# EternityJune25/ComoRAG

Measured on NVIDIA H100. Metric: queries/sec, higher is better.
Workload: dtype bf16

## Files before the change

### comorag_b200/csrc/gemm.cu

```cuda
#include <cstdlib>

#include "common.cuh"
#include "gemm.cuh"
#include "ptx.cuh"

namespace crag {

constexpr int kGemmBM = 128;
constexpr int kGemmBN = 128;
constexpr int kGemmBK = 64;
constexpr int kGemmConsumerWarps = 8;
constexpr int kGemmThreads = 32 * kGemmConsumerWarps + 32;
constexpr int kGemmStages = 3;

struct GemmLayout {
  static constexpr int kABytes = kGemmBM * kGemmBK * 2;
  static constexpr int kBBytes = kGemmBN * kGemmBK * 2;
  static constexpr int kStageBytes = kABytes + kBBytes;
  static constexpr size_t smem_bytes() { return 1024 + size_t(kGemmStages) * kStageBytes + 2 * kGemmStages * 8; }
};

__device__ __forceinline__ float gelu_erf(float x) {
  const float z = x * 0.70710678118654752f;
  const float az = fabsf(z);
  float t;
  asm("rcp.approx.ftz.f32 %0, %1;" : "=f"(t) : "f"(fmaf(0.3275911f, az, 1.0f)));
  float p = fmaf(1.061405429f, t, -1.453152027f);
  p = fmaf(p, t, 1.421413741f);
  p = fmaf(p, t, -0.284496736f);
  p = fmaf(p, t, 0.254829592f);
  p *= t;
  float e;
  asm("ex2.approx.ftz.f32 %0, %1;" : "=f"(e) : "f"(az * az * -1.4426950408889634f));
  const float erf_abs = fmaf(-p, e, 1.0f);
  const float half_x = 0.5f * x;
  return fmaf(half_x, copysignf(erf_abs, z), half_x);
}

__device__ __forceinline__ uint32_t pack_bf16x2(float a, float b) {
  __nv_bfloat162 v = __floats2bfloat162_rn(a, b);
  return *reinterpret_cast<uint32_t*>(&v);
}

template <int EPI>
__global__ void __launch_bounds__(kGemmThreads, 2)
gemm_bf16_kernel(const __grid_constant__ CUtensorMap tm_a, const __grid_constant__ CUtensorMap tm_b, int M, int N,
                 int K, const float* __restrict__ bias, const __nv_bfloat16* __restrict__ residual, int64_t ldr,
                 __nv_bfloat16* __restrict__ out, int64_t ldo) {
  using L = GemmLayout;
  constexpr int STAGES = kGemmStages;
  extern __shared__ uint8_t smem_raw[];
  uint8_t* smem = reinterpret_cast<uint8_t*>((reinterpret_cast<uintptr_t>(smem_raw) + 1023) & ~uintptr_t(1023));
  uint64_t* bar_full = reinterpret_cast<uint64_t*>(smem + STAGES * L::kStageBytes);
  uint64_t* bar_empty = bar_full + STAGES;

  const int warp = threadIdx.x >> 5;
  const int lane = threadIdx.x & 31;
  const int n_blk = blockIdx.x, m_blk = blockIdx.y;
  const int num_kb = (K + kGemmBK - 1) / kGemmBK;

  if (threadIdx.x == 0) {
    for (int s = 0; s < STAGES; ++s) {
      mbar_init(&bar_full[s], 1);
      mbar_init(&bar_empty[s], kGemmConsumerWarps);
    }
    fence_mbar_init();
  }
  __syncthreads();

  if (warp == kGemmConsumerWarps) {
    if (lane == 0) {
      tma_prefetch_desc(&tm_a);
      tma_prefetch_desc(&tm_b);
      const uint64_t pol_w = policy_evict_last();
      int stage = 0;
      uint32_t phase = 0;
      for (int kb = 0; kb < num_kb; ++kb) {
        mbar_wait(&bar_empty[stage], phase ^ 1);
        uint8_t* sa = smem + stage * L::kStageBytes;
        mbar_arrive_expect_tx(&bar_full[stage], L::kStageBytes);
        tma_load_2d(&tm_a, &bar_full[stage], sa, kb * kGemmBK, m_blk * kGemmBM);
        tma_load_2d_hint(&tm_b, &bar_full[stage], sa + L::kABytes, kb * kGemmBK, n_blk * kGemmBN, pol_w);
        if (++stage == STAGES) { stage = 0; phase ^= 1; }
      }
    }
    return;
  }

  const int wg = warp >> 2;
  float acc[kGemmBN / 2];
#pragma unroll
  for (int i = 0; i < kGemmBN / 2; ++i) acc[i] = 0.f;
  int stage = 0, prev = 0;
  uint32_t phase = 0;
  for (int kb = 0; kb < num_kb; ++kb) {
    mbar_wait(&bar_full[stage], phase);
    const uint32_t a_addr = smem_u32(smem + stage * L::kStageBytes) + wg * 64 * 128;
    const uint32_t b_addr = smem_u32(smem + stage * L::kStageBytes + L::kABytes);
    wgmma_fence();
#pragma unroll
    for (int ks = 0; ks < kGemmBK / 16; ++ks)
      wgmma_m64n128k16_ss(acc, wgmma_desc_sw128(a_addr + ks * 32), wgmma_desc_sw128(b_addr + ks * 32), 1u);
    wgmma_commit();
    wgmma_wait<1>();
    if (kb > 0 && lane == 0) mbar_arrive(&bar_empty[prev]);
    prev = stage;
    if (++stage == STAGES) { stage = 0; phase ^= 1; }
  }
  wgmma_wait<0>();
  wgmma_fence_regs(acc);

  const int row0 = m_blk * kGemmBM + wg * 64 + (warp & 3) * 16 + (lane >> 2);
  const int col0 = n_blk * kGemmBN + 2 * (lane & 3);
#pragma unroll
  for (int j = 0; j < kGemmBN / 8; ++j) {
    const int col = col0 + 8 * j;
    if (col >= N) continue;
    const float2 b = __ldg(reinterpret_cast<const float2*>(bias + col));
#pragma unroll
    for (int h = 0; h < 2; ++h) {
      const int row = row0 + 8 * h;
      if (row >= M) continue;
      float x0 = acc[4 * j + 2 * h] + b.x, x1 = acc[4 * j + 2 * h + 1] + b.y;
      if (EPI == GEMM_EPI_BIAS_GELU) {
        x0 = gelu_erf(x0);
        x1 = gelu_erf(x1);
      }
      if (EPI == GEMM_EPI_BIAS_RESIDUAL) {
        const __nv_bfloat162 r = *reinterpret_cast<const __nv_bfloat162*>(residual + int64_t(row) * ldr + col);
        x0 += __bfloat162float(r.x);
        x1 += __bfloat162float(r.y);
      }
      *reinterpret_cast<uint32_t*>(out + int64_t(row) * ldo + col) = pack_bf16x2(x0, x1);
    }
  }
}

template <int EPI>
static int launch_gemm_t(const CUtensorMap& tm_a, const CUtensorMap& tm_b, int M, int N, int K, const float* bias,
                         const __nv_bfloat16* residual, int64_t ldr, __nv_bfloat16* out, int64_t ldo,
                         cudaStream_t stream) {
  auto kern = gemm_bf16_kernel<EPI>;
  {
    static bool done[64] = {false};
    int dev = 0;
    CRAG_CUDA_OK(cudaGetDevice(&dev));
    if (dev < 0 || dev >= 64 || !done[dev]) {
      CRAG_CUDA_OK(cudaFuncSetAttribute(kern, cudaFuncAttributeMaxDynamicSharedMemorySize, int(GemmLayout::smem_bytes())));
      if (dev >= 0 && dev < 64) done[dev] = true;
    }
  }
  const dim3 grid((N + kGemmBN - 1) / kGemmBN, (M + kGemmBM - 1) / kGemmBM);
  kern<<<grid, kGemmThreads, GemmLayout::smem_bytes(), stream>>>(tm_a, tm_b, M, N, K, bias, residual, ldr, out, ldo);
  CRAG_CUDA_OK(cudaGetLastError());
  return CRAG_OK;
}

int gemm_bf16(const void* a, int64_t lda, const void* w, int64_t ldw, const float* bias, const void* residual,
              int64_t ldr, void* out, int64_t ldo, int M, int N, int K, int epi, cudaStream_t stream) {
  if (M <= 0) return CRAG_OK;
  if (N < 8 || K < 8 || N % 8 != 0 || K % 8 != 0) return fail(CRAG_ERR_INVALID, "gemm: N and K must be positive multiples of 8 (N=%d K=%d)", N, K);
  if (lda % 8 || ldw % 8 || ldo % 8 || (epi == GEMM_EPI_BIAS_RESIDUAL && ldr % 8)) return fail(CRAG_ERR_INVALID, "gemm: leading dimensions must be multiples of 8 elements");
  if (!a || !w || !bias || !out || (epi == GEMM_EPI_BIAS_RESIDUAL && !residual)) return fail(CRAG_ERR_INVALID, "gemm: null pointer");
  if ((uintptr_t(a) | uintptr_t(w) | uintptr_t(out) | uintptr_t(bias) | uintptr_t(residual)) & 15) return fail(CRAG_ERR_INVALID, "gemm: pointers must be 16-byte aligned");
  if ((M + kGemmBM - 1) / kGemmBM > 65535) return fail(CRAG_ERR_INVALID, "gemm: M too large (%d)", M);
  const __nv_bfloat16* res = static_cast<const __nv_bfloat16*>(residual);
  __nv_bfloat16* o = static_cast<__nv_bfloat16*>(out);
  CUtensorMap tm_a, tm_b;
  int rc = make_tmap_bf16_2d(&tm_a, a, uint64_t(M), uint64_t(K), uint64_t(lda) * 2, kGemmBM);
  if (rc != CRAG_OK) return rc;
  rc = make_tmap_bf16_2d(&tm_b, w, uint64_t(N), uint64_t(K), uint64_t(ldw) * 2, kGemmBN);
  if (rc != CRAG_OK) return rc;
  switch (epi) {
    case GEMM_EPI_BIAS: return launch_gemm_t<GEMM_EPI_BIAS>(tm_a, tm_b, M, N, K, bias, res, ldr, o, ldo, stream);
    case GEMM_EPI_BIAS_GELU: return launch_gemm_t<GEMM_EPI_BIAS_GELU>(tm_a, tm_b, M, N, K, bias, res, ldr, o, ldo, stream);
    case GEMM_EPI_BIAS_RESIDUAL: return launch_gemm_t<GEMM_EPI_BIAS_RESIDUAL>(tm_a, tm_b, M, N, K, bias, res, ldr, o, ldo, stream);
  }
  return fail(CRAG_ERR_INVALID, "gemm: unknown epilogue %d", epi);
}

}

extern "C" int crag_gemm_bf16(const void* a, int64_t lda, const void* w, int64_t ldw, const float* bias,
                              const void* residual, int64_t ldr, void* out, int64_t ldo, int m, int n, int k,
                              int epilogue, crag_stream_t stream) {
  return crag::gemm_bf16(a, lda, w, ldw, bias, residual, ldr, out, ldo, m, n, k, epilogue,
                         static_cast<cudaStream_t>(stream));
}
```

### comorag_b200/csrc/ptx.cuh

```cuda
#pragma once
#include <cuda.h>
#include <cuda_runtime.h>
#include <cuda_bf16.h>
#include <stdint.h>

namespace crag {

__device__ __forceinline__ uint32_t smem_u32(const void* p) {
  return static_cast<uint32_t>(__cvta_generic_to_shared(p));
}

__device__ __forceinline__ bool elect_one() {
  uint32_t pred = 0;
  asm volatile(
      "{\n\t.reg .pred p;\n\t"
      "elect.sync _|p, 0xffffffff;\n\t"
      "selp.u32 %0, 1, 0, p;\n\t}"
      : "=r"(pred));
  return pred != 0;
}

__device__ __forceinline__ void mbar_init(uint64_t* bar, uint32_t count) {
  asm volatile("mbarrier.init.shared::cta.b64 [%0], %1;" ::"r"(smem_u32(bar)), "r"(count));
}
__device__ __forceinline__ void fence_mbar_init() {
  asm volatile("fence.mbarrier_init.release.cluster;" ::: "memory");
}
__device__ __forceinline__ void fence_proxy_async() {
  asm volatile("fence.proxy.async.shared::cta;" ::: "memory");
}
__device__ __forceinline__ void mbar_arrive_expect_tx(uint64_t* bar, uint32_t bytes) {
  asm volatile("mbarrier.arrive.expect_tx.shared::cta.b64 _, [%0], %1;" ::"r"(smem_u32(bar)), "r"(bytes)
               : "memory");
}
__device__ __forceinline__ void mbar_arrive(uint64_t* bar) {
  asm volatile("mbarrier.arrive.shared::cta.b64 _, [%0];" ::"r"(smem_u32(bar)) : "memory");
}
__device__ __forceinline__ bool mbar_try_wait(uint64_t* bar, uint32_t parity) {
  uint32_t ok;
  asm volatile(
      "{\n\t.reg .pred p;\n\t"
      "mbarrier.try_wait.parity.shared::cta.b64 p, [%1], %2;\n\t"
      "selp.u32 %0, 1, 0, p;\n\t}"
      : "=r"(ok)
      : "r"(smem_u32(bar)), "r"(parity)
      : "memory");
  return ok != 0;
}
#ifndef CRAG_MBAR_SPIN_LIMIT
#define CRAG_MBAR_SPIN_LIMIT (1ll << 33)
#endif
__device__ __forceinline__ void mbar_wait(uint64_t* bar, uint32_t parity) {
  if (mbar_try_wait(bar, parity)) return;
  const long long t0 = clock64();
  uint32_t spins = 0;
  while (!mbar_try_wait(bar, parity)) {
    if ((++spins & 0x3FF) == 0 && clock64() - t0 > CRAG_MBAR_SPIN_LIMIT) __trap();
  }
}

__device__ __forceinline__ void tma_prefetch_desc(const CUtensorMap* m) {
  asm volatile("prefetch.tensormap [%0];" ::"l"(reinterpret_cast<uint64_t>(m)) : "memory");
}
__device__ __forceinline__ void tma_load_2d(const CUtensorMap* m, uint64_t* bar, void* dst, int32_t c0,
                                            int32_t c1) {
  asm volatile(
      "cp.async.bulk.tensor.2d.shared::cluster.global.mbarrier::complete_tx::bytes"
      " [%0], [%1, {%3, %4}], [%2];" ::"r"(smem_u32(dst)),
      "l"(reinterpret_cast<uint64_t>(m)), "r"(smem_u32(bar)), "r"(c0), "r"(c1)
      : "memory");
}
__device__ __forceinline__ void tma_load_2d_hint(const CUtensorMap* m, uint64_t* bar, void* dst, int32_t c0,
                                                 int32_t c1, uint64_t policy) {
  asm volatile(
      "cp.async.bulk.tensor.2d.shared::cluster.global.mbarrier::complete_tx::bytes.L2::cache_hint"
      " [%0], [%1, {%3, %4}], [%2], %5;" ::"r"(smem_u32(dst)),
      "l"(reinterpret_cast<uint64_t>(m)), "r"(smem_u32(bar)), "r"(c0), "r"(c1), "l"(policy)
      : "memory");
}
__device__ __forceinline__ uint64_t policy_evict_first() {
  uint64_t p;
  asm volatile("createpolicy.fractional.L2::evict_first.b64 %0, 1.0;" : "=l"(p));
  return p;
}
__device__ __forceinline__ uint64_t policy_evict_normal() {
  uint64_t p;
  asm volatile("createpolicy.fractional.L2::evict_normal.b64 %0, 1.0;" : "=l"(p));
  return p;
}
__device__ __forceinline__ uint64_t policy_evict_last() {
  uint64_t p;
  asm volatile("createpolicy.fractional.L2::evict_last.b64 %0, 1.0;" : "=l"(p));
  return p;
}

__device__ __forceinline__ void wgmma_fence() { asm volatile("wgmma.fence.sync.aligned;" ::: "memory"); }
__device__ __forceinline__ void wgmma_commit() { asm volatile("wgmma.commit_group.sync.aligned;" ::: "memory"); }
template <int N>
__device__ __forceinline__ void wgmma_wait() { asm volatile("wgmma.wait_group.sync.aligned %0;" ::"n"(N) : "memory"); }
template <int R>
__device__ __forceinline__ void wgmma_fence_regs(float (&d)[R]) {
#pragma unroll
  for (int i = 0; i < R; ++i) asm volatile("" : "+f"(d[i])::"memory");
}

__device__ __forceinline__ uint64_t wgmma_desc_sw128(uint32_t smem_addr) {
  uint64_t d = 0;
  d |= static_cast<uint64_t>((smem_addr & 0x3FFFF) >> 4);
  d |= static_cast<uint64_t>(1) << 16;
  d |= static_cast<uint64_t>(1024 >> 4) << 32;
  d |= static_cast<uint64_t>(1) << 62;
  return d;
}

__device__ __forceinline__ void wgmma_m64n32k16_ss(float (&d)[16], uint64_t desc_a, uint64_t desc_b, uint32_t accumulate) {
  asm volatile(
      "{\n\t.reg .pred p;\n\t"
      "setp.ne.b32 p, %18, 0;\n\t"
      "wgmma.mma_async.sync.aligned.m64n32k16.f32.bf16.bf16 "
      "{%0, %1, %2, %3, %4, %5, %6, %7, %8, %9, %10, %11, %12, %13, %14, %15}, %16, %17, p, 1, 1, 0, 0;\n\t}"
      : "+f"(d[0]), "+f"(d[1]), "+f"(d[2]), "+f"(d[3]), "+f"(d[4]), "+f"(d[5]), "+f"(d[6]), "+f"(d[7]), "+f"(d[8]), "+f"(d[9]), "+f"(d[10]), "+f"(d[11]), "+f"(d[12]), "+f"(d[13]), "+f"(d[14]), "+f"(d[15])
      : "l"(desc_a), "l"(desc_b), "r"(accumulate));
}
__device__ __forceinline__ void wgmma_m64n64k16_ss(float (&d)[32], uint64_t desc_a, uint64_t desc_b, uint32_t accumulate) {
  asm volatile(
      "{\n\t.reg .pred p;\n\t"
      "setp.ne.b32 p, %34, 0;\n\t"
      "wgmma.mma_async.sync.aligned.m64n64k16.f32.bf16.bf16 "
      "{%0, %1, %2, %3, %4, %5, %6, %7, %8, %9, %10, %11, %12, %13, %14, %15, %16, %17, %18, %19, %20, %21, %22, %23, %24, %25, %26, %27, %28, %29, %30, %31}, %32, %33, p, 1, 1, 0, 0;\n\t}"
      : "+f"(d[0]), "+f"(d[1]), "+f"(d[2]), "+f"(d[3]), "+f"(d[4]), "+f"(d[5]), "+f"(d[6]), "+f"(d[7]), "+f"(d[8]), "+f"(d[9]), "+f"(d[10]), "+f"(d[11]), "+f"(d[12]), "+f"(d[13]), "+f"(d[14]), "+f"(d[15]), "+f"(d[16]), "+f"(d[17]), "+f"(d[18]), "+f"(d[19]), "+f"(d[20]), "+f"(d[21]), "+f"(d[22]), "+f"(d[23]), "+f"(d[24]), "+f"(d[25]), "+f"(d[26]), "+f"(d[27]), "+f"(d[28]), "+f"(d[29]), "+f"(d[30]), "+f"(d[31])
      : "l"(desc_a), "l"(desc_b), "r"(accumulate));
}
__device__ __forceinline__ void wgmma_m64n128k16_ss(float (&d)[64], uint64_t desc_a, uint64_t desc_b, uint32_t accumulate) {
  asm volatile(
      "{\n\t.reg .pred p;\n\t"
      "setp.ne.b32 p, %66, 0;\n\t"
      "wgmma.mma_async.sync.aligned.m64n128k16.f32.bf16.bf16 "
      "{%0, %1, %2, %3, %4, %5, %6, %7, %8, %9, %10, %11, %12, %13, %14, %15, %16, %17, %18, %19, %20, %21, %22, %23, %24, %25, %26, %27, %28, %29, %30, %31, %32, %33, %34, %35, %36, %37, %38, %39, %40, %41, %42, %43, %44, %45, %46, %47, %48, %49, %50, %51, %52, %53, %54, %55, %56, %57, %58, %59, %60, %61, %62, %63}, %64, %65, p, 1, 1, 0, 0;\n\t}"
      : "+f"(d[0]), "+f"(d[1]), "+f"(d[2]), "+f"(d[3]), "+f"(d[4]), "+f"(d[5]), "+f"(d[6]), "+f"(d[7]), "+f"(d[8]), "+f"(d[9]), "+f"(d[10]), "+f"(d[11]), "+f"(d[12]), "+f"(d[13]), "+f"(d[14]), "+f"(d[15]), "+f"(d[16]), "+f"(d[17]), "+f"(d[18]), "+f"(d[19]), "+f"(d[20]), "+f"(d[21]), "+f"(d[22]), "+f"(d[23]), "+f"(d[24]), "+f"(d[25]), "+f"(d[26]), "+f"(d[27]), "+f"(d[28]), "+f"(d[29]), "+f"(d[30]), "+f"(d[31]), "+f"(d[32]), "+f"(d[33]), "+f"(d[34]), "+f"(d[35]), "+f"(d[36]), "+f"(d[37]), "+f"(d[38]), "+f"(d[39]), "+f"(d[40]), "+f"(d[41]), "+f"(d[42]), "+f"(d[43]), "+f"(d[44]), "+f"(d[45]), "+f"(d[46]), "+f"(d[47]), "+f"(d[48]), "+f"(d[49]), "+f"(d[50]), "+f"(d[51]), "+f"(d[52]), "+f"(d[53]), "+f"(d[54]), "+f"(d[55]), "+f"(d[56]), "+f"(d[57]), "+f"(d[58]), "+f"(d[59]), "+f"(d[60]), "+f"(d[61]), "+f"(d[62]), "+f"(d[63])
      : "l"(desc_a), "l"(desc_b), "r"(accumulate));
}
__device__ __forceinline__ void wgmma_m64n64k16_rs_bmn(float (&d)[32], const uint32_t (&a)[4], uint64_t desc_b,
                                                      uint32_t accumulate) {
  asm volatile(
      "{\n\t.reg .pred p;\n\t"
      "setp.ne.b32 p, %37, 0;\n\t"
      "wgmma.mma_async.sync.aligned.m64n64k16.f32.bf16.bf16 "
      "{%0, %1, %2, %3, %4, %5, %6, %7, %8, %9, %10, %11, %12, %13, %14, %15, %16, %17, %18, %19, %20, %21, %22, %23, %24, %25, %26, %27, %28, %29, %30, %31}, {%32, %33, %34, %35}, %36, p, 1, 1, 1;\n\t}"
      : "+f"(d[0]), "+f"(d[1]), "+f"(d[2]), "+f"(d[3]), "+f"(d[4]), "+f"(d[5]), "+f"(d[6]), "+f"(d[7]), "+f"(d[8]), "+f"(d[9]), "+f"(d[10]), "+f"(d[11]), "+f"(d[12]), "+f"(d[13]), "+f"(d[14]), "+f"(d[15]), "+f"(d[16]), "+f"(d[17]), "+f"(d[18]), "+f"(d[19]), "+f"(d[20]), "+f"(d[21]), "+f"(d[22]), "+f"(d[23]), "+f"(d[24]), "+f"(d[25]), "+f"(d[26]), "+f"(d[27]), "+f"(d[28]), "+f"(d[29]), "+f"(d[30]), "+f"(d[31])
      : "r"(a[0]), "r"(a[1]), "r"(a[2]), "r"(a[3]), "l"(desc_b), "r"(accumulate));
}

__device__ __forceinline__ void named_bar_sync(uint32_t id, uint32_t nthreads) {
  asm volatile("barrier.cta.sync %0, %1;" ::"r"(id), "r"(nthreads) : "memory");
}
__device__ __forceinline__ bool named_bar_or(uint32_t id, uint32_t nthreads, bool pred) {
  uint32_t out;
  asm volatile(
      "{\n\t.reg .pred p, q;\n\t"
      "setp.ne.b32 p, %1, 0;\n\t"
      "barrier.cta.red.or.pred q, %2, %3, p;\n\t"
      "selp.u32 %0, 1, 0, q;\n\t}"
      : "=r"(out)
      : "r"(static_cast<uint32_t>(pred)), "r"(id), "r"(nthreads)
      : "memory");
  return out != 0;
}

}
```

Baseline: 4611.

## Add persistent warp-specialized 128x256 GEMM with TMA-store epilogue for large problems

Adds a persistent GEMM kernel with 128x256 tiles, used when the wide tile count is at least the SM count. It uses a grouped-M tile order for L2 reuse, register reallocation between the producer and the two consumer warpgroups, and an epilogue that stages output in swizzled shared memory, writes it with TMA stores, and TMA-loads the residual. The aim is better wgmma efficiency and operand reuse, lower launch and tail overhead, and less uncoalesced epilogue traffic. It costs one CTA per SM, heavy register pressure from 128 accumulators, and no overlap between the epilogue and the next tile's MMA within a warpgroup.

Result: no change. 4606 (median of 6 runs) (-0.1%).

```diff
diff --git a/comorag_b200/csrc/gemm.cu b/comorag_b200/csrc/gemm.cu
--- a/comorag_b200/csrc/gemm.cu
+++ b/comorag_b200/csrc/gemm.cu
@@ -136,6 +136,192 @@
   }
 }
 
+constexpr int kWideBN = 256;
+constexpr int kWideStages = 3;
+constexpr int kWideThreads = 384;
+constexpr int kGemmGroupM = 16;
+
+struct WideLayout {
+  static constexpr int kABytes = kGemmBM * kGemmBK * 2;
+  static constexpr int kBBytes = kWideBN * kGemmBK * 2;
+  static constexpr int kStageBytes = kABytes + kBBytes;
+  static constexpr int kOutBoxBytes = 64 * 64 * 2;
+  static constexpr int kOutBytes = 4 * kOutBoxBytes;
+  static constexpr int kOutOffset = kWideStages * kStageBytes;
+  static constexpr int kBarOffset = kOutOffset + 2 * kOutBytes;
+  static constexpr size_t smem_bytes() { return 1024 + size_t(kBarOffset) + (2 * kWideStages + 2) * 8; }
+};
+
+template <int EPI>
+__global__ void __launch_bounds__(kWideThreads, 1)
+gemm_bf16_persistent_kernel(const __grid_constant__ CUtensorMap tm_a, const __grid_constant__ CUtensorMap tm_b,
+                            const __grid_constant__ CUtensorMap tm_out, const __grid_constant__ CUtensorMap tm_res,
+                            int M, int N, int K, const float* __restrict__ bias) {
+  using L = WideLayout;
+  constexpr int STAGES = kWideStages;
+  extern __shared__ uint8_t smem_raw[];
+  uint8_t* smem = reinterpret_cast<uint8_t*>((reinterpret_cast<uintptr_t>(smem_raw) + 1023) & ~uintptr_t(1023));
+  uint64_t* bar_full = reinterpret_cast<uint64_t*>(smem + L::kBarOffset);
+  uint64_t* bar_empty = bar_full + STAGES;
+  uint64_t* bar_res = bar_empty + STAGES;
+
+  const int warp = threadIdx.x >> 5;
+  const int lane = threadIdx.x & 31;
+  const int num_kb = (K + kGemmBK - 1) / kGemmBK;
+  const int tiles_m = (M + kGemmBM - 1) / kGemmBM;
+  const int tiles_n = (N + kWideBN - 1) / kWideBN;
+  const int num_tiles = tiles_m * tiles_n;
+  auto tile_coords = [&](int tile, int& m_blk, int& n_blk) {
+    const int group = tile / (kGemmGroupM * tiles_n);
+    const int first_m = group * kGemmGroupM;
+    const int group_m = min(kGemmGroupM, tiles_m - first_m);
+    const int in_group = tile - group * kGemmGroupM * tiles_n;
+    m_blk = first_m + in_group % group_m;
+    n_blk = in_group / group_m;
+  };
+
+  if (threadIdx.x == 0) {
+    for (int s = 0; s < STAGES; ++s) {
+      mbar_init(&bar_full[s], 1);
+      mbar_init(&bar_empty[s], kGemmConsumerWarps);
+    }
+    mbar_init(&bar_res[0], 1);
+    mbar_init(&bar_res[1], 1);
+    fence_mbar_init();
+  }
+  __syncthreads();
+
+  if (warp < 4) {
+    setmaxnreg_dec<40>();
+    if (warp == 0 && lane == 0) {
+      tma_prefetch_desc(&tm_a);
+      tma_prefetch_desc(&tm_b);
+      const uint64_t pol_w = policy_evict_last();
+      int stage = 0;
+      uint32_t phase = 0;
+      for (int tile = blockIdx.x; tile < num_tiles; tile += gridDim.x) {
+        int m_blk, n_blk;
+        tile_coords(tile, m_blk, n_blk);
+        for (int kb = 0; kb < num_kb; ++kb) {
+          mbar_wait(&bar_empty[stage], phase ^ 1);
+          uint8_t* sa = smem + stage * L::kStageBytes;
+          mbar_arrive_expect_tx(&bar_full[stage], L::kStageBytes);
+          tma_load_2d(&tm_a, &bar_full[stage], sa, kb * kGemmBK, m_blk * kGemmBM);
+          tma_load_2d_hint(&tm_b, &bar_full[stage], sa + L::kABytes, kb * kGemmBK, n_blk * kWideBN, pol_w);
+          if (++stage == STAGES) { stage = 0; phase ^= 1; }
+        }
+      }
+    }
+    return;
+  }
+
+  setmaxnreg_inc<232>();
+  const int wg = (warp >> 2) - 1;
+  const bool leader = (threadIdx.x & 127) == 0;
+  uint8_t* out_tile = smem + L::kOutOffset + wg * L::kOutBytes;
+  const int frag_row = (warp & 3) * 16 + (lane >> 2);
+  const uint32_t frag_off = frag_row * 128 + 4 * (lane & 3);
+  const uint32_t swz = lane >> 2;
+  if (leader) {
+    tma_prefetch_desc(&tm_out);
+    if (EPI == GEMM_EPI_BIAS_RESIDUAL) tma_prefetch_desc(&tm_res);
+  }
+  int stage = 0;
+  uint32_t phase = 0, res_phase = 0;
+  float acc[kWideBN / 2];
+  for (int tile = blockIdx.x; tile < num_tiles; tile += gridDim.x) {
+    int m_blk, n_blk;
+    tile_coords(tile, m_blk, n_blk);
+    const int row0 = m_blk * kGemmBM + wg * 64, col0 = n_blk * kWideBN;
+    if (leader) {
+      bulk_wait_group_read<0>();
+      if (EPI == GEMM_EPI_BIAS_RESIDUAL) {
+        mbar_arrive_expect_tx(&bar_res[wg], L::kOutBytes);
+#pragma unroll
+        for (int b = 0; b < 4; ++b) tma_load_2d(&tm_res, &bar_res[wg], out_tile + b * L::kOutBoxBytes, col0 + 64 * b, row0);
+      }
+    }
+#pragma unroll
+    for (int i = 0; i < kWideBN / 2; ++i) acc[i] = 0.f;
+    int prev = 0;
+    for (int kb = 0; kb < num_kb; ++kb) {
+      mbar_wait(&bar_full[stage], phase);
+      const uint32_t a_addr = smem_u32(smem + stage * L::kStageBytes) + wg * 64 * 128;
+      const uint32_t b_addr = smem_u32(smem + stage * L::kStageBytes + L::kABytes);
+      wgmma_fence();
+#pragma unroll
+      for (int ks = 0; ks < kGemmBK / 16; ++ks)
+        wgmma_m64n256k16_ss(acc, wgmma_desc_sw128(a_addr + ks * 32), wgmma_desc_sw128(b_addr + ks * 32), 1u);
+      wgmma_commit();
+      wgmma_wait<1>();
+      if (kb > 0 && lane == 0) mbar_arrive(&bar_empty[prev]);
+      prev = stage;
+      if (++stage == STAGES) { stage = 0; phase ^= 1; }
+    }
+    wgmma_wait<0>();
+    wgmma_fence_regs(acc);
+    if (lane == 0) mbar_arrive(&bar_empty[prev]);
+
+    if (EPI == GEMM_EPI_BIAS_RESIDUAL) {
+      mbar_wait(&bar_res[wg], res_phase);
+      res_phase ^= 1;
+    } else {
+      named_bar_sync(1 + wg, 128);
+    }
+    const uint32_t out_base = smem_u32(out_tile) + frag_off;
+#pragma unroll
+    for (int j = 0; j < kWideBN / 8; ++j) {
+      const int col = col0 + 8 * j + 2 * (lane & 3);
+      const float2 b = col < N ? __ldg(reinterpret_cast<const float2*>(bias + col)) : make_float2(0.f, 0.f);
+      const uint32_t addr = out_base + (j >> 3) * L::kOutBoxBytes + (((j & 7) ^ swz) << 4);
+#pragma unroll
+      for (int h = 0; h < 2; ++h) {
+        float x0 = acc[4 * j + 2 * h] + b.x, x1 = acc[4 * j + 2 * h + 1] + b.y;
+        if (EPI == GEMM_EPI_BIAS_GELU) {
+          x0 = gelu_erf(x0);
+          x1 = gelu_erf(x1);
+        }
+        if (EPI == GEMM_EPI_BIAS_RESIDUAL) {
+          uint32_t rv;
+          asm volatile("ld.shared.b32 %0, [%1];" : "=r"(rv) : "r"(addr + h * 8 * 128));
+          const __nv_bfloat162 r = *reinterpret_cast<const __nv_bfloat162*>(&rv);
+          x0 += __bfloat162float(r.x);
+          x1 += __bfloat162float(r.y);
+        }
+        asm volatile("st.shared.b32 [%0], %1;" ::"r"(addr + h * 8 * 128), "r"(pack_bf16x2(x0, x1)) : "memory");
+      }
+    }
+    fence_proxy_async();
+    named_bar_sync(1 + wg, 128);
+    if (leader) {
+#pragma unroll
+      for (int b = 0; b < 4; ++b) tma_store_2d(&tm_out, out_tile + b * L::kOutBoxBytes, col0 + 64 * b, row0);
+      bulk_commit_group();
+    }
+  }
+  if (leader) bulk_wait_group_read<0>();
+}
+
+template <int EPI>
+static int launch_gemm_wide_t(const CUtensorMap& tm_a, const CUtensorMap& tm_b, const CUtensorMap& tm_out,
+                              const CUtensorMap& tm_res, int M, int N, int K, const float* bias, int num_tiles,
+                              int sms, cudaStream_t stream) {
+  auto kern = gemm_bf16_persistent_kernel<EPI>;
+  {
+    static bool done[64] = {false};
+    int dev = 0;
+    CRAG_CUDA_OK(cudaGetDevice(&dev));
+    if (dev < 0 || dev >= 64 || !done[dev]) {
+      CRAG_CUDA_OK(cudaFuncSetAttribute(kern, cudaFuncAttributeMaxDynamicSharedMemorySize, int(WideLayout::smem_bytes())));
+      if (dev >= 0 && dev < 64) done[dev] = true;
+    }
+  }
+  kern<<<min(num_tiles, sms), kWideThreads, WideLayout::smem_bytes(), stream>>>(tm_a, tm_b, tm_out, tm_res, M, N, K,
+                                                                               bias);
+  CRAG_CUDA_OK(cudaGetLastError());
+  return CRAG_OK;
+}
+
 template <int EPI>
 static int launch_gemm_t(const CUtensorMap& tm_a, const CUtensorMap& tm_b, int M, int N, int K, const float* bias,
                          const __nv_bfloat16* residual, int64_t ldr, __nv_bfloat16* out, int64_t ldo,
@@ -169,6 +355,27 @@
   CUtensorMap tm_a, tm_b;
   int rc = make_tmap_bf16_2d(&tm_a, a, uint64_t(M), uint64_t(K), uint64_t(lda) * 2, kGemmBM);
   if (rc != CRAG_OK) return rc;
+  const int sms = sm_count();
+  if (sms <= 0) return CRAG_ERR_CUDA;
+  const int wide_tiles = ((M + kGemmBM - 1) / kGemmBM) * ((N + kWideBN - 1) / kWideBN);
+  if (wide_tiles >= sms) {
+    CUtensorMap tm_out, tm_res;
+    rc = make_tmap_bf16_2d(&tm_b, w, uint64_t(N), uint64_t(K), uint64_t(ldw) * 2, kWideBN);
+    if (rc != CRAG_OK) return rc;
+    rc = make_tmap_bf16_2d(&tm_out, out, uint64_t(M), uint64_t(N), uint64_t(ldo) * 2, 64);
+    if (rc != CRAG_OK) return rc;
+    tm_res = tm_out;
+    if (epi == GEMM_EPI_BIAS_RESIDUAL) {
+      rc = make_tmap_bf16_2d(&tm_res, residual, uint64_t(M), uint64_t(N), uint64_t(ldr) * 2, 64);
+      if (rc != CRAG_OK) return rc;
+    }
+    switch (epi) {
+      case GEMM_EPI_BIAS: return launch_gemm_wide_t<GEMM_EPI_BIAS>(tm_a, tm_b, tm_out, tm_res, M, N, K, bias, wide_tiles, sms, stream);
+      case GEMM_EPI_BIAS_GELU: return launch_gemm_wide_t<GEMM_EPI_BIAS_GELU>(tm_a, tm_b, tm_out, tm_res, M, N, K, bias, wide_tiles, sms, stream);
+      case GEMM_EPI_BIAS_RESIDUAL: return launch_gemm_wide_t<GEMM_EPI_BIAS_RESIDUAL>(tm_a, tm_b, tm_out, tm_res, M, N, K, bias, wide_tiles, sms, stream);
+    }
+    return fail(CRAG_ERR_INVALID, "gemm: unknown epilogue %d", epi);
+  }
   rc = make_tmap_bf16_2d(&tm_b, w, uint64_t(N), uint64_t(K), uint64_t(ldw) * 2, kGemmBN);
   if (rc != CRAG_OK) return rc;
   switch (epi) {
diff --git a/comorag_b200/csrc/ptx.cuh b/comorag_b200/csrc/ptx.cuh
--- a/comorag_b200/csrc/ptx.cuh
+++ b/comorag_b200/csrc/ptx.cuh
@@ -78,6 +78,23 @@
       "l"(reinterpret_cast<uint64_t>(m)), "r"(smem_u32(bar)), "r"(c0), "r"(c1), "l"(policy)
       : "memory");
 }
+__device__ __forceinline__ void tma_store_2d(const CUtensorMap* m, const void* src, int32_t c0, int32_t c1) {
+  asm volatile("cp.async.bulk.tensor.2d.global.shared::cta.bulk_group [%0, {%2, %3}], [%1];" ::"l"(
+                   reinterpret_cast<uint64_t>(m)),
+               "r"(smem_u32(src)), "r"(c0), "r"(c1)
+               : "memory");
+}
+__device__ __forceinline__ void bulk_commit_group() { asm volatile("cp.async.bulk.commit_group;" ::: "memory"); }
+template <int N>
+__device__ __forceinline__ void bulk_wait_group_read() {
+  asm volatile("cp.async.bulk.wait_group.read %0;" ::"n"(N) : "memory");
+}
+
+template <int R>
+__device__ __forceinline__ void setmaxnreg_dec() { asm volatile("setmaxnreg.dec.sync.aligned.u32 %0;" ::"n"(R)); }
+template <int R>
+__device__ __forceinline__ void setmaxnreg_inc() { asm volatile("setmaxnreg.inc.sync.aligned.u32 %0;" ::"n"(R)); }
+
 __device__ __forceinline__ uint64_t policy_evict_first() {
   uint64_t p;
   asm volatile("createpolicy.fractional.L2::evict_first.b64 %0, 1.0;" : "=l"(p));
@@ -140,6 +157,15 @@
       : "+f"(d[0]), "+f"(d[1]), "+f"(d[2]), "+f"(d[3]), "+f"(d[4]), "+f"(d[5]), "+f"(d[6]), "+f"(d[7]), "+f"(d[8]), "+f"(d[9]), "+f"(d[10]), "+f"(d[11]), "+f"(d[12]), "+f"(d[13]), "+f"(d[14]), "+f"(d[15]), "+f"(d[16]), "+f"(d[17]), "+f"(d[18]), "+f"(d[19]), "+f"(d[20]), "+f"(d[21]), "+f"(d[22]), "+f"(d[23]), "+f"(d[24]), "+f"(d[25]), "+f"(d[26]), "+f"(d[27]), "+f"(d[28]), "+f"(d[29]), "+f"(d[30]), "+f"(d[31]), "+f"(d[32]), "+f"(d[33]), "+f"(d[34]), "+f"(d[35]), "+f"(d[36]), "+f"(d[37]), "+f"(d[38]), "+f"(d[39]), "+f"(d[40]), "+f"(d[41]), "+f"(d[42]), "+f"(d[43]), "+f"(d[44]), "+f"(d[45]), "+f"(d[46]), "+f"(d[47]), "+f"(d[48]), "+f"(d[49]), "+f"(d[50]), "+f"(d[51]), "+f"(d[52]), "+f"(d[53]), "+f"(d[54]), "+f"(d[55]), "+f"(d[56]), "+f"(d[57]), "+f"(d[58]), "+f"(d[59]), "+f"(d[60]), "+f"(d[61]), "+f"(d[62]), "+f"(d[63])
       : "l"(desc_a), "l"(desc_b), "r"(accumulate));
 }
+__device__ __forceinline__ void wgmma_m64n256k16_ss(float (&d)[128], uint64_t desc_a, uint64_t desc_b, uint32_t accumulate) {
+  asm volatile(
+      "{\n\t.reg .pred p;\n\t"
+      "setp.ne.b32 p, %130, 0;\n\t"
+      "wgmma.mma_async.sync.aligned.m64n256k16.f32.bf16.bf16 "
+      "{%0, %1, %2, %3, %4, %5, %6, %7, %8, %9, %10, %11, %12, %13, %14, %15, %16, %17, %18, %19, %20, %21, %22, %23, %24, %25, %26, %27, %28, %29, %30, %31, %32, %33, %34, %35, %36, %37, %38, %39, %40, %41, %42, %43, %44, %45, %46, %47, %48, %49, %50, %51, %52, %53, %54, %55, %56, %57, %58, %59, %60, %61, %62, %63, %64, %65, %66, %67, %68, %69, %70, %71, %72, %73, %74, %75, %76, %77, %78, %79, %80, %81, %82, %83, %84, %85, %86, %87, %88, %89, %90, %91, %92, %93, %94, %95, %96, %97, %98, %99, %100, %101, %102, %103, %104, %105, %106, %107, %108, %109, %110, %111, %112, %113, %114, %115, %116, %117, %118, %119, %120, %121, %122, %123, %124, %125, %126, %127}, %128, %129, p, 1, 1, 0, 0;\n\t}"
+      : "+f"(d[0]), "+f"(d[1]), "+f"(d[2]), "+f"(d[3]), "+f"(d[4]), "+f"(d[5]), "+f"(d[6]), "+f"(d[7]), "+f"(d[8]), "+f"(d[9]), "+f"(d[10]), "+f"(d[11]), "+f"(d[12]), "+f"(d[13]), "+f"(d[14]), "+f"(d[15]), "+f"(d[16]), "+f"(d[17]), "+f"(d[18]), "+f"(d[19]), "+f"(d[20]), "+f"(d[21]), "+f"(d[22]), "+f"(d[23]), "+f"(d[24]), "+f"(d[25]), "+f"(d[26]), "+f"(d[27]), "+f"(d[28]), "+f"(d[29]), "+f"(d[30]), "+f"(d[31]), "+f"(d[32]), "+f"(d[33]), "+f"(d[34]), "+f"(d[35]), "+f"(d[36]), "+f"(d[37]), "+f"(d[38]), "+f"(d[39]), "+f"(d[40]), "+f"(d[41]), "+f"(d[42]), "+f"(d[43]), "+f"(d[44]), "+f"(d[45]), "+f"(d[46]), "+f"(d[47]), "+f"(d[48]), "+f"(d[49]), "+f"(d[50]), "+f"(d[51]), "+f"(d[52]), "+f"(d[53]), "+f"(d[54]), "+f"(d[55]), "+f"(d[56]), "+f"(d[57]), "+f"(d[58]), "+f"(d[59]), "+f"(d[60]), "+f"(d[61]), "+f"(d[62]), "+f"(d[63]), "+f"(d[64]), "+f"(d[65]), "+f"(d[66]), "+f"(d[67]), "+f"(d[68]), "+f"(d[69]), "+f"(d[70]), "+f"(d[71]), "+f"(d[72]), "+f"(d[73]), "+f"(d[74]), "+f"(d[75]), "+f"(d[76]), "+f"(d[77]), "+f"(d[78]), "+f"(d[79]), "+f"(d[80]), "+f"(d[81]), "+f"(d[82]), "+f"(d[83]), "+f"(d[84]), "+f"(d[85]), "+f"(d[86]), "+f"(d[87]), "+f"(d[88]), "+f"(d[89]), "+f"(d[90]), "+f"(d[91]), "+f"(d[92]), "+f"(d[93]), "+f"(d[94]), "+f"(d[95]), "+f"(d[96]), "+f"(d[97]), "+f"(d[98]), "+f"(d[99]), "+f"(d[100]), "+f"(d[101]), "+f"(d[102]), "+f"(d[103]), "+f"(d[104]), "+f"(d[105]), "+f"(d[106]), "+f"(d[107]), "+f"(d[108]), "+f"(d[109]), "+f"(d[110]), "+f"(d[111]), "+f"(d[112]), "+f"(d[113]), "+f"(d[114]), "+f"(d[115]), "+f"(d[116]), "+f"(d[117]), "+f"(d[118]), "+f"(d[119]), "+f"(d[120]), "+f"(d[121]), "+f"(d[122]), "+f"(d[123]), "+f"(d[124]), "+f"(d[125]), "+f"(d[126]), "+f"(d[127])
+      : "l"(desc_a), "l"(desc_b), "r"(accumulate));
+}
 __device__ __forceinline__ void wgmma_m64n64k16_rs_bmn(float (&d)[32], const uint32_t (&a)[4], uint64_t desc_b,
                                                       uint32_t accumulate) {
   asm volatile(
```
